# ina-foss/inaSpeechSegmenter

Measured on AMD Instinct MI355X. Metric: hours-of-audio segmented/sec (smn+gender, 16 kHz mono), higher is better.
Workload: dtype f32 (f16x3 split-operand MFMA, f32 accumulate; f64 FFT)

## Files before the change

inaspeechsegmenter_amd/_native.py:

```python
import ctypes as C
import os

import numpy as np

_HERE = os.path.dirname(os.path.abspath(__file__))
LIB_PATH = os.environ.get('ISS_LIB') or os.path.join(_HERE, 'libiss_hip.so')

PROG_COLS = 32
OP_CONV, OP_POOL, OP_SOFTMAX, OP_STATPOOL, OP_ACT, OP_ELT = 1, 2, 3, 4, 5, 6
(ELT_COPY, ELT_ADD, ELT_SUB, ELT_MUL, ELT_MAX, ELT_MIN, ELT_AVG, ELT_ZERO, ELT_PERMUTE) = range(9)
(C_OP, C_IN, C_OUT, C_RES, C_H, C_W, C_CIN, C_HO, C_WO, C_COUT, C_KH, C_KW, C_SH, C_SW, C_PT, C_PL,
 C_ACT, C_WOFF, C_BOFF, C_PSOFF, C_PTOFF, C_INMODE, C_POOLKIND, C_ORDER, C_FPOOLH, C_FPOOLW, C_DUALW, C_DUALB, C_ACTPARAM, C_ACTPARAM2, C_ACTPARAM3) = range(31)
PREC_BF16X3, PREC_F32, PREC_F16X3 = 0, 1, 2
K_ALIGN = 32
BUF_INPUT = -2
MAX_NETS = 8
RS_JOB = np.dtype([('src_offset', '<i8'), ('frames_in', '<i8'), ('channels', '<i4'), ('format', '<i4'), ('filter', '<i4'),
                   ('reserved', '<i4'), ('dst_offset', '<i8'), ('frames_out', '<i8')])
RS_FORMAT = {np.dtype(np.uint8): 0, np.dtype('<i2'): 1, np.dtype('<i4'): 2, np.dtype('<f4'): 3, np.dtype('<f8'): 4}
RS_I8, RS_ULAW, RS_ALAW, RS_SWAP = 8, 9, 10, 0x100
ADPCM_JOB = np.dtype([('src_offset', '<i8'), ('block_begin', '<i8'), ('nblocks', '<i8'), ('frames_total', '<i8'), ('channels', '<i4'),
                      ('block_align', '<i4'), ('output', '<i4'), ('filter', '<i4'), ('dst_offset', '<i8'), ('frames_out', '<i8')])
ADPCM_TO_SIGNAL, ADPCM_TO_STAGE = 0, 1
ADPCM_STATUS = {1: 'step index above 88', 2: 'predictor index above 6'}
# ... 145 lines not shown
        'iss_survey_geometry': (C.c_int, [pi32, pi32, pi32]),
        'iss_survey_stats': (C.c_int, [vp, pi64, pi64]),
        'iss_get_signal_pcm16': (C.c_int, [vp, pi16, i64, i64]),
        'iss_resample_stats': (C.c_int, [vp, pi64, pi64]),
        'iss_flac_index': (C.c_int, [vp, i64, i64, vp, vp, i64, pi64, pi64, C.c_char_p, i32]),
        'iss_flac_crc': (C.c_int, [vp, i64, pi32, pi32]),
        'iss_flac_decode_host': (C.c_int, [vp, i64, vp, i64, i32, i32, i64, vp, pi32]),
        'iss_flac_decode': (C.c_int, [vp, vp, i64, vp, i64, vp, i32, i64, pi32]),
        'iss_flac_get_stage': (C.c_int, [vp, i32, vp, i64]),
        'iss_flac_stats': (C.c_int, [vp, pi64, pi64]),
        'iss_adpcm_decode_host': (C.c_int, [vp, i64, i64, i32, i32, i64, pi16, pi32]),
        'iss_adpcm_decode': (C.c_int, [vp, vp, i64, vp, i32, i64, i64, pi32]),
        'iss_adpcm_get_stage': (C.c_int, [vp, i32, vp, i64]),
        'iss_adpcm_stats': (C.c_int, [vp, pi64, pi64]),
        'iss_msadpcm_decode_host': (C.c_int, [vp, i64, i64, i32, i32, i64, pi16, pi32]),
        'iss_msadpcm_decode': (C.c_int, [vp, vp, i64, vp, i32, i64, i64, pi32]),
        'iss_msadpcm_get_stage': (C.c_int, [vp, i32, vp, i64]),
        'iss_msadpcm_stats': (C.c_int, [vp, pi64, pi64]),
        'iss_host_alloc': (C.c_int, [vp, C.c_size_t, C.POINTER(vp)]),
        'iss_host_free': (C.c_int, [vp, vp]),
        'iss_cnn_probs_async': (C.c_int, [vp, C.c_int, pi32, i32, pf, pu8, pi64]),
        'iss_cnn_dead_stats': (C.c_int, [vp, pi64, pi64]),
        'iss_wait': (C.c_int, [vp, i64]),
        'iss_comm_unique_id': (C.c_int, [vp, pu8]),
        'iss_comm_init': (C.c_int, [vp, pu8, i32, i32]),
        'iss_comm_destroy': (C.c_int, [vp]),
        'iss_allgather_segments': (C.c_int, [vp, pi32, i32, i32, pi32, pi32]),
        'iss_comm_allreduce_max': (C.c_int, [vp, pd]),
        'iss_comm_info': (C.c_int, [vp, pi32, pi32, pi32, C.c_char_p, i32]),
        'iss_sidekit': (C.c_int, [vp, pi32]),
        'iss_get_loge': (C.c_int, [vp, pf]),
        'iss_get_mspec': (C.c_int, [vp, pf]),
        'iss_set_mspec': (C.c_int, [vp, pf, i32]),
        'iss_cnn_load': (C.c_int, [vp, C.c_int, pi32, i32, pf, i64, i32, pi64, i32, i32, i32, i32]),
        'iss_cnn_load_shared': (C.c_int, [vp, C.c_int, C.c_int, pi32, i32, i32, pi64, i32, i32, i32, i32]),
        'iss_cnn_probs': (C.c_int, [vp, C.c_int, pi32, i32, pf, pu8]),
        'iss_cnn_forward': (C.c_int, [vp, C.c_int, pf, i32, pf]),
        'iss_cnn_flops': (C.c_int, [vp, C.c_int, pd]),
        'iss_set_precision': (C.c_int, [vp, C.c_int]),
        'iss_set_precision_guard': (C.c_int, [vp, C.c_float]),
        'iss_cnn_precision_info': (C.c_int, [vp, C.c_int, pi32, pf, pi32, pi32, pf]),
        'iss_cnn_set_net_precision': (C.c_int, [vp, C.c_int, C.c_int]),
        'iss_vbx_tables': (C.c_int, [vp, pd, pd]),
        'iss_vbx_features': (C.c_int, [vp, pi32, pd, i64, pf, pi32]),
        'iss_vbx_set_dither': (C.c_int, [vp, pd, i64]),
        'iss_vbx_features_pcm16': (C.c_int, [vp, pi16, i64, pf, pi32]),
# ... 478 lines not shown
        return probs, fin.astype(bool)

    def cnn_probs_async(self, net_id, win_row, probs_out=None, finite_out=None):
        wr = np.ascontiguousarray(win_row, dtype=np.int32)
        n = wr.size
        if probs_out is None:
            probs_out = np.empty((n, self._net_out[net_id]), dtype=np.float32)
        if finite_out is None:
            finite_out = np.empty(n, dtype=np.uint8)
        assert probs_out.size >= n * self._net_out[net_id] and finite_out.size >= n
        t = C.c_int64(-1)
        self._ck(self._L.iss_cnn_probs_async(self._h, net_id, _ptr(wr, C.c_int32), n, _ptr(probs_out, C.c_float),
                                             _ptr(finite_out, C.c_uint8), C.byref(t)), 'iss_cnn_probs_async')
        return t.value, probs_out, finite_out

    def cnn_dead_stats(self):
        w, d = C.c_int64(0), C.c_int64(0)
        self._ck(self._L.iss_cnn_dead_stats(self._h, C.byref(w), C.byref(d)), 'iss_cnn_dead_stats')
        return {'windows': w.value, 'dead': d.value}

    def wait(self, ticket=-1):
        self._ck(self._L.iss_wait(self._h, int(ticket)), 'iss_wait')

    def comm_unique_id(self):
        buf = np.zeros(128, dtype=np.uint8)
        self._ck(self._L.iss_comm_unique_id(self._h, _ptr(buf, C.c_uint8)), 'iss_comm_unique_id')
        return buf.tobytes()

    def comm_init(self, uid, rank, world):
        buf = np.frombuffer(bytes(uid), dtype=np.uint8).copy()
        assert buf.size == 128
        self._ck(self._L.iss_comm_init(self._h, _ptr(buf, C.c_uint8), int(rank), int(world)), 'iss_comm_init')
        self.comm_rank, self.comm_world = int(rank), int(world)

    def comm_destroy(self):
        self._ck(self._L.iss_comm_destroy(self._h), 'iss_comm_destroy')
        self.comm_rank, self.comm_world = 0, 1

    def allgather_segments(self, rows, capacity):
        world = self.comm_world
        out = np.zeros((world, capacity, 4), dtype=np.int32)
        counts = np.zeros(world, dtype=np.int32)
        if rows is None:
            rows, n = np.zeros((1, 4), np.int32), -1
        else:
            rows = np.ascontiguousarray(rows, dtype=np.int32).reshape(-1, 4)
# ... 180 lines not shown
```

inaspeechsegmenter_amd/csrc/cnn.hip:

```cpp
#include "conv_select.h"

using namespace issk;

namespace {

template <int MODE>
__global__ __launch_bounds__(256) void conv_igemm_kernel(const ConvArgs p) {
    __shared__ __attribute__((aligned(16))) float sA[2][BM * LDK];
    __shared__ __attribute__((aligned(16))) float sB[2][BN * LDK];

    const int tid = threadIdx.x, lane = tid & 63, wv = tid >> 6;
    unsigned mt, nt;
    gemm_tile_of_block(blockIdx.x, p.nblk, p.nblk_n, mt, nt);
    const long long m0 = (long long)mt * BM;
    const int n0 = (int)nt * BN;

    const int k4 = tid & 3;
    const int lr = tid >> 2;
    RowSrc rs[2];
#pragma unroll
    for (int j = 0; j < 2; ++j) rs[j] = row_source<MODE>(p, m0 + lr + 64 * j);
    const int bn = n0 + lr;
    const bool bok = bn < p.Cout;
    const float* wrow = p.w + (size_t)(bok ? bn : 0) * p.Kpad + k4 * 4;
// ... 852 lines not shown
    if (i < n) p[i] = 0.5f;
}

__global__ void mask_probs_kernel(float* probs, const uint8_t* finite, long long n, int C) {
    const long long i = (long long)blockIdx.x * blockDim.x + threadIdx.x;
    if (i < n * C && !finite[i / C]) probs[i] = 0.5f;
}

__global__ __launch_bounds__(256) void row_flags_kernel(const float* __restrict__ mspec, int T, uint8_t* __restrict__ flag) {
    const int t = blockIdx.x * 256 + threadIdx.x;
    if (t >= T) return;
    float v[24];
#pragma unroll
    for (int k = 0; k < 6; ++k) *reinterpret_cast<float4*>(v + 4 * k) = reinterpret_cast<const float4*>(mspec + (size_t)t * 24)[k];
    flag[t] = (uint8_t)iss_row_flag(v);
}

__global__ void scatter_probs_kernel(const float* __restrict__ res, const uint8_t* __restrict__ lfinite, const int32_t* __restrict__ map,
                                     long long n, int C, float* __restrict__ out, uint8_t* __restrict__ finite) {
    const long long i = (long long)blockIdx.x * blockDim.x + threadIdx.x;
    if (i >= n * C) return;
    const long long r = i / C;
    const int k = (int)(i - r * C);
    const long long m = map[r];
    const uint8_t f = lfinite[r];
    out[m * C + k] = f ? res[i] : 0.5f;
    if (k == 0) finite[m] = f;
}

inline int roundup(int a, int b) { return (a + b - 1) / b * b; }

inline uint16_t bf16_rne(float x) {
    uint32_t u;
    memcpy(&u, &x, 4);
    u += 0x7fffu + ((u >> 16) & 1u);
    return (uint16_t)(u >> 16);
}
inline float bf16_to_f32(uint16_t h) {
    uint32_t u = (uint32_t)h << 16;
    float x;
    memcpy(&x, &u, 4);
    return x;
}

}

IssParamArrays::~IssParamArrays() {
// ... 727 lines not shown
    int chosen = eff;
    if (rc == ISS_OK) probe(eff, worst);
    const double first = worst;
    if (rc == ISS_OK && worst > (double)c->guard_threshold) {
        chosen = ISS_PREC_F32;
        const int other = eff == ISS_PREC_BF16X3 ? ISS_PREC_F16X3 : ISS_PREC_BF16X3;
        if (other == ISS_PREC_BF16X3 || n.f16_ok) {
            double w2 = 0.0;
            probe(other, w2);
            if (rc == ISS_OK && w2 <= (double)c->guard_threshold) { chosen = other; worst = w2; }
        }
    }
    c->in_guard = false;
    n.prec_override = -1;
    if (rc != ISS_OK) return rc;
    if (compared == 0) { n.guard_slots = 0; return ISS_OK; }
    n.guard_dlogp = (float)std::min(first, 1e30); n.guard_slots = compared;
    n.guard_dlogp_chosen = chosen == eff ? n.guard_dlogp : (chosen == ISS_PREC_F32 ? 0.f : (float)worst);
    if (chosen != eff) { n.prec_override = chosen; n.guard_state = ISS_GUARD_ESCALATED; }
    else n.guard_state = ISS_GUARD_PASSED;
    return ISS_OK;
}

static int ensure_row_flags(iss_ctx* c) {
    if (c->flags_epoch == c->feat_epoch) return ISS_OK;
    int rc;
    if ((rc = iss_reserve(c, c->d_rowflag, (size_t)c->T))) return rc;
    if ((rc = iss_rowflag_host(c, (size_t)c->T))) return rc;
    iss_prof_begin(c, 2, 0);
    hipLaunchKernelGGL(row_flags_kernel, dim3((c->T + 255) / 256), dim3(256), 0, c->stream, (const float*)c->mspec.p, (int)c->T,
                       (uint8_t*)c->d_rowflag.p);
    iss_prof_end(c);
    ISS_HIP(c, hipGetLastError());
    ISS_HIP(c, hipMemcpyAsync(c->h_rowflag, c->d_rowflag.p, (size_t)c->T, hipMemcpyDeviceToHost, c->stream));
    ISS_HIP(c, hipStreamSynchronize(c->stream));
    c->bad_prefix.clear();
    c->flags_epoch = c->feat_epoch;
    return ISS_OK;
}

static const std::vector<int32_t>& bad_prefix(iss_ctx* c, int w) {
    std::vector<int32_t>& P = c->bad_prefix[w];
    if (P.size() != (size_t)c->T + 1) {
        P.resize((size_t)c->T + 1);
        P[0] = 0;
        for (int32_t t = 0; t < c->T; ++t) P[t + 1] = P[t] + (c->h_rowflag[t] < w ? 1 : 0);
    }
    return P;
}

extern "C" int iss_cnn_dead_stats(iss_ctx* c, int64_t* windows, int64_t* dead) {
    if (!c) return ISS_EINVAL;
    if (windows) *windows = c->win_total;
    if (dead) *dead = c->win_dead;
    return ISS_OK;
}

static int cnn_probs_impl(iss_ctx* c, int id, const int32_t* win_row, int32_t nslots, float* probs_out,
                          uint8_t* finite_out, bool async, int64_t* ticket_out) {
    if (!c) return ISS_EINVAL;
    if (ticket_out) *ticket_out = -1;
// ... 28 lines not shown
    const bool compact = nlive < nslots;
    const int32_t* rows = compact ? lm.data() : win_row;
    if (!c->in_guard && n.guard_state == ISS_GUARD_PENDING && nlive > 0 && (rc = precision_guard(c, id, rows, nlive))) return rc;
    const size_t nup = compact ? 2 * (size_t)nlive : (size_t)nslots;
    if ((rc = iss_reserve(c, c->d_winrow, (nup ? nup : 1) * 4))) return rc;
    if ((rc = iss_reserve(c, c->d_stats, (size_t)nslots * 8))) return rc;
    if ((rc = iss_reserve(c, c->d_finite, (size_t)nslots))) return rc;
    if (compact && (rc = iss_reserve(c, c->d_lfinite, (size_t)(nlive ? nlive : 1)))) return rc;
    if ((rc = iss_reserve(c, c->d_out, (size_t)nslots * n.out_dim * 4))) return rc;
    int bc = 0;
    if (nlive > 0 && (rc = plan_chunk(c, n, nlive, &bc))) return rc;
    if (nup == 0) {
    } else if (async || compact) {
        void* pinned; int slot;
        if ((rc = iss_stage_host(c, rows, nup * 4, &pinned, &slot))) return rc;
        ISS_HIP(c, hipMemcpyAsync(c->d_winrow.p, pinned, nup * 4, hipMemcpyHostToDevice, c->stream));
        iss_stage_mark(c, slot);
    } else {
        ISS_HIP(c, hipMemcpyAsync(c->d_winrow.p, win_row, (size_t)nslots * 4, hipMemcpyHostToDevice, c->stream));
    }
    const int32_t* d_map = (const int32_t*)c->d_winrow.p + nlive;
    uint8_t* d_fin = compact ? (uint8_t*)c->d_lfinite.p : (uint8_t*)c->d_finite.p;
    const long long tot = (long long)nslots * n.out_dim;
    if (compact) {
        iss_prof_begin(c, 2, 0);
        hipLaunchKernelGGL(fill_half_kernel, dim3((unsigned)((tot + 255) / 256)), dim3(256), 0, c->stream, (float*)c->d_out.p, tot);
        iss_prof_end(c);
        ISS_HIP(c, hipGetLastError());
        ISS_HIP(c, hipMemsetAsync(c->d_finite.p, 0, (size_t)nslots, c->stream));
    }
    if (nlive > 0) {
        iss_prof_begin(c, 2, 0);
        hipLaunchKernelGGL(patch_stats_kernel, dim3((nlive + 3) / 4), dim3(256), 0, c->stream, (const float*)c->mspec.p,
                           (const int32_t*)c->d_winrow.p, nlive, n.in_w, (float*)c->d_stats.p, d_fin);
        iss_prof_end(c);
        ISS_HIP(c, hipGetLastError());
    }
    bool share = !(c->diag & ISS_DIAG_NO_SHARED_FIRST);
    if (nlive > 0) {
        int gmin = rows[0], gmax = rows[0];
        for (int i = 1; i < nlive; ++i) { gmin = std::min(gmin, rows[i]); gmax = std::max(gmax, rows[i]); }
        if ((long long)(gmax - gmin + 68) * 4 > (long long)nlive * 68) share = false;
    }
    for (int s0 = 0; s0 < nlive; s0 += bc) {
        const int cur = std::min(bc, nlive - s0);
        float* res = nullptr;
        int rmin = rows[s0], rmax = rows[s0];
        for (int i = s0 + 1; i < s0 + cur; ++i) { rmin = std::min(rmin, rows[i]); rmax = std::max(rmax, rows[i]); }
        rc = run_program(c, n, cur, (const int32_t*)c->d_winrow.p + s0, (const float*)c->d_stats.p + 2 * (size_t)s0,
                         (const uint8_t*)d_fin + s0, nullptr, &res, rmin, rmax, share);
        if (rc) return rc;
        if (compact) {
            const long long ct = (long long)cur * n.out_dim;
            iss_prof_begin(c, 2, 0);
            hipLaunchKernelGGL(scatter_probs_kernel, dim3((unsigned)((ct + 255) / 256)), dim3(256), 0, c->stream, (const float*)res,
                               (const uint8_t*)d_fin + s0, d_map + s0, (long long)cur, n.out_dim, (float*)c->d_out.p, (uint8_t*)c->d_finite.p);
            iss_prof_end(c);
            ISS_HIP(c, hipGetLastError());
        } else {
            ISS_HIP(c, hipMemcpyAsync((float*)c->d_out.p + (size_t)s0 * n.out_dim, res, (size_t)cur * n.out_dim * 4,
                                      hipMemcpyDeviceToDevice, c->stream));
        }
    }
    if (!compact) {
        hipLaunchKernelGGL(mask_probs_kernel, dim3((unsigned)((tot + 255) / 256)), dim3(256), 0, c->stream,
                           (float*)c->d_out.p, (const uint8_t*)c->d_finite.p, (long long)nslots, n.out_dim);
        ISS_HIP(c, hipGetLastError());
    }
    ISS_HIP(c, hipMemcpyAsync(probs_out, c->d_out.p, (size_t)tot * 4, hipMemcpyDeviceToHost, c->stream));
    ISS_HIP(c, hipMemcpyAsync(finite_out, c->d_finite.p, (size_t)nslots, hipMemcpyDeviceToHost, c->stream));
    if (async) {
        hipEvent_t ev;
        if (!c->ev_pool.empty()) { ev = c->ev_pool.back(); c->ev_pool.pop_back(); }
        else ISS_HIP(c, hipEventCreate(&ev));
        ISS_HIP(c, hipEventRecord(ev, c->stream));
        c->ticket_ev.push_back(ev);
        if (ticket_out) *ticket_out = c->ticket_base + (int64_t)c->ticket_ev.size() - 1;
        return ISS_OK;
    }
    ISS_HIP(c, hipStreamSynchronize(c->stream));
    iss_prof_collect(c);
    return ISS_OK;
}

extern "C" int iss_cnn_probs(iss_ctx* c, int id, const int32_t* win_row, int32_t nslots, float* probs_out,
                             uint8_t* finite_out) {
    return cnn_probs_impl(c, id, win_row, nslots, probs_out, finite_out, false, nullptr);
}

extern "C" int iss_cnn_probs_async(iss_ctx* c, int id, const int32_t* win_row, int32_t nslots, float* probs_out,
                                   uint8_t* finite_out, int64_t* ticket_out) {
    return cnn_probs_impl(c, id, win_row, nslots, probs_out, finite_out, true, ticket_out);
}

extern "C" int iss_cnn_forward(iss_ctx* c, int id, const float* x, int32_t nsamp, float* out) {
    if (!c) return ISS_EINVAL;
    if (id < 0 || id >= ISS_MAX_NETS || nsamp < 0 || (nsamp > 0 && (!x || !out)))
        return iss_fail(c, ISS_EINVAL, "iss_cnn_forward: bad argument");
    IssNet& n = c->nets[id];
    if (!n.loaded) return iss_fail(c, ISS_ESTATE, "iss_cnn_forward: net %d not loaded", id);
// ... 57 lines not shown
```

inaspeechsegmenter_amd/csrc/iss_core.cpp:

```cpp
#include "iss_internal.h"
#include <cstring>
#include <cmath>
#include <mutex>

static std::string g_err;
static std::mutex g_err_mu;

int iss_fail(iss_ctx* c, int code, const char* fmt, ...) {
    char buf[1024];
    va_list ap;
    va_start(ap, fmt);
    vsnprintf(buf, sizeof(buf), fmt, ap);
    va_end(ap);
    if (c) c->err = buf;
    else { std::lock_guard<std::mutex> l(g_err_mu); g_err = buf; }
    return code;
}

int iss_reserve(iss_ctx* c, DevBuf& b, size_t bytes) {
    if (bytes <= b.cap) return ISS_OK;
    if (b.p) { ISS_HIP(c, hipStreamSynchronize(c->stream)); ISS_HIP(c, hipFree(b.p)); b.p = nullptr; b.cap = 0; }
    size_t want = bytes + (bytes >> 3) + 256;
    hipError_t e = hipMalloc(&b.p, want);
    if (e != hipSuccess) {
// ... 38 lines not shown
    *out = c;
    return ISS_OK;
}

static void free_buf(DevBuf& b) { if (b.p) (void)hipFree(b.p); b.p = nullptr; b.cap = 0; }

extern "C" void iss_destroy(iss_ctx* c) {
    if (!c) return;
    (void)hipSetDevice(c->device);
    if (c->stream) (void)hipStreamSynchronize(c->stream);
    for (int i = 0; i < ISS_MAX_NETS; ++i) iss_cnn_free(c, i);
    void* singles[] = {c->d_window, c->d_melw, c->d_mellim, c->d_tw, c->d_vbx_window, c->d_vbx_melw, c->d_vbx_mellim};
    for (void* p : singles) if (p) (void)hipFree(p);
    DevBuf* bufs[] = {&c->sig, &c->mspec, &c->loge, &c->d_winrow, &c->d_stats, &c->d_finite, &c->d_out, &c->d_in, &c->raw1, &c->d_rowflag, &c->d_lfinite,
                      &c->vbx_sig, &c->vbx_dither, &c->vbx_fb, &c->vbx_out, &c->vbx_meta, &c->rs_src, &c->rs_jobs, &c->sv_src, &c->sv_jobs, &c->sv_ws, &c->sv_res,
                      &c->flac.src, &c->flac.rows, &c->flac.status, &c->flac.stage,
                      &c->adpcm.src, &c->adpcm.rows, &c->adpcm.status, &c->adpcm.stage,
                      &c->msadpcm.src, &c->msadpcm.rows, &c->msadpcm.status, &c->msadpcm.stage};
    for (DevBuf* b : bufs) free_buf(*b);
    for (auto& b : c->act) free_buf(b);
    for (auto& f : c->rs_filters) if (f.d_taps) (void)hipFree(f.d_taps);
    for (auto& p : c->pending) { (void)hipEventDestroy(p.a); (void)hipEventDestroy(p.b); }
    for (auto& e : c->ev_pool) (void)hipEventDestroy(e);
    for (auto& e : c->ticket_ev) (void)hipEventDestroy(e);
    for (auto& s : c->staging) { if (s.p) (void)hipHostFree(s.p); if (s.done) (void)hipEventDestroy(s.done); }
    if (c->order_ev) (void)hipEventDestroy(c->order_ev);
    if (c->h_rowflag) (void)hipHostFree(c->h_rowflag);
    iss_comm_destroy(c);
    free_buf(c->comm_send); free_buf(c->comm_recv);
    if (c->stream) (void)hipStreamDestroy(c->stream);
    delete c;
}

extern "C" int iss_set_workspace_limit(iss_ctx* c, uint64_t bytes) {
    if (!c) return ISS_EINVAL;
    if (bytes < (64ull << 20)) return iss_fail(c, ISS_EINVAL, "workspace limit below 64 MiB");
    c->ws_limit = bytes;
    return ISS_OK;
}

extern "C" int iss_synchronize(iss_ctx* c) {
    if (!c) return ISS_EINVAL;
    ISS_HIP(c, hipSetDevice(c->device));
    ISS_HIP(c, hipStreamSynchronize(c->stream));
    return ISS_OK;
}

extern "C" int iss_scribble(iss_ctx* c, uint32_t word) {
    if (!c) return ISS_EINVAL;
    ISS_HIP(c, hipSetDevice(c->device));
    ISS_HIP(c, hipStreamSynchronize(c->stream));
    std::vector<DevBuf*> bufs = {&c->raw1, &c->d_stats, &c->d_finite, &c->d_lfinite, &c->d_out, &c->d_in, &c->d_winrow, &c->d_rowflag,
                                 &c->vbx_fb, &c->vbx_meta, &c->vbx_sig, &c->rs_src, &c->rs_jobs, &c->sv_src, &c->sv_jobs, &c->sv_ws, &c->sv_res,
                                 &c->flac.src, &c->flac.rows, &c->flac.status, &c->flac.stage,
                                 &c->adpcm.src, &c->adpcm.rows, &c->adpcm.status, &c->adpcm.stage,
                                 &c->msadpcm.src, &c->msadpcm.rows, &c->msadpcm.status, &c->msadpcm.stage};
    for (auto& b : c->act) bufs.push_back(&b);
    for (DevBuf* b : bufs) {
        if (!b->p) continue;
        if (b->cap >= 4) ISS_HIP(c, hipMemsetD32Async((hipDeviceptr_t)b->p, (int)word, b->cap / 4, c->stream));
        for (size_t i = b->cap & ~(size_t)3; i < b->cap; ++i)
            ISS_HIP(c, hipMemsetD8Async((hipDeviceptr_t)((char*)b->p + i), (unsigned char)(word >> (8 * (i & 3))), 1, c->stream));
    }
    c->flags_epoch = 0;
    c->bad_prefix.clear();
    c->sv_held.id = c->flac.held = c->adpcm.held = c->msadpcm.held = 0;
    return ISS_OK;
}

extern "C" int iss_sidekit_tables(iss_ctx* c, const double* window400, const float* bank) {
    if (!c || !window400 || !bank) return iss_fail(c, ISS_EINVAL, "iss_sidekit_tables: NULL argument");
    ISS_HIP(c, hipSetDevice(c->device));
    std::vector<int32_t> lim(24 * 3);
    std::vector<float> w;
    for (int f = 0; f < 24; ++f) {
        int lo = -1, hi = -1;
        for (int k = 0; k < 257; ++k)
            if (bank[f * 257 + k] != 0.0f) { if (lo < 0) lo = k; hi = k; }
        if (lo < 0) { lo = 0; hi = -1; }
        if (hi >= 256) return iss_fail(c, ISS_EINVAL, "mel filter %d touches bin 256; unsupported table", f);
        lim[f * 3 + 0] = lo; lim[f * 3 + 1] = hi - lo + 1; lim[f * 3 + 2] = (int32_t)w.size();
        for (int k = lo; k <= hi; ++k) w.push_back(bank[f * 257 + k]);
    }
    if (w.size() > 1024) return iss_fail(c, ISS_EINVAL, "mel bank has %zu weights (>1024)", w.size());
    std::vector<double> tw(2 * 256 * 2);
    for (int k = 0; k < 256; ++k) {
        tw[2 * k] = cos(-2.0 * M_PI * k / 256.0);       tw[2 * k + 1] = sin(-2.0 * M_PI * k / 256.0);
// ... 102 lines not shown
    memcpy(c->staging[slot].p, src, bytes);
    *pinned_out = c->staging[slot].p;
    *slot_out = slot;
    return ISS_OK;
}
int iss_rowflag_host(iss_ctx* c, size_t rows) {
    if (rows <= c->h_rowflag_cap) return ISS_OK;
    if (c->h_rowflag) { ISS_HIP(c, hipStreamSynchronize(c->stream)); (void)hipHostFree(c->h_rowflag); c->h_rowflag = nullptr; c->h_rowflag_cap = 0; }
    const size_t want = rows + (rows >> 2) + 4096;
    hipError_t e = hipHostMalloc((void**)&c->h_rowflag, want, hipHostMallocDefault);
    if (e != hipSuccess) { c->h_rowflag = nullptr; return iss_fail(c, ISS_ENOMEM, "hipHostMalloc(%zu) failed: %s", want, hipGetErrorString(e)); }
    c->h_rowflag_cap = want;
    return ISS_OK;
}
void iss_stage_mark(iss_ctx* c, int slot) {
    auto& s = c->staging[slot];
    (void)hipEventRecord(s.done, c->stream);
    s.busy = true;
}

extern "C" int iss_wait(iss_ctx* c, int64_t ticket) {
    if (!c) return ISS_EINVAL;
    ISS_HIP(c, hipSetDevice(c->device));
    const int64_t last = c->ticket_base + (int64_t)c->ticket_ev.size() - 1;
    if (ticket < 0 || ticket >= last) {
        ISS_HIP(c, hipStreamSynchronize(c->stream));
        for (auto e : c->ticket_ev) c->ev_pool.push_back(e);
        c->ticket_base += (int64_t)c->ticket_ev.size();
        c->ticket_ev.clear();
        iss_prof_collect(c);
        return ISS_OK;
    }
    if (ticket < c->ticket_base) return ISS_OK;
    ISS_HIP(c, hipEventSynchronize(c->ticket_ev[(size_t)(ticket - c->ticket_base)]));
    return ISS_OK;
}

extern "C" int iss_sidekit(iss_ctx* c, int32_t* T_out) {
    if (!c) return ISS_EINVAL;
    if (!c->sk_tables) return iss_fail(c, ISS_ESTATE, "iss_sidekit: call iss_sidekit_tables first");
    if (c->sig_kind == 0) return iss_fail(c, ISS_ESTATE, "iss_sidekit: no resident signal");
    ISS_HIP(c, hipSetDevice(c->device));
    int64_t n = c->sig_n;
    int64_t T = n >= 400 ? (n - 400) / 160 + 1 : 0;
    if (T > 0x7fffffffLL / 24) return iss_fail(c, ISS_EINVAL, "signal too long (%lld frames)", (long long)T);
    c->T = (int32_t)T;
    int rc = iss_reserve(c, c->mspec, (size_t)(T > 0 ? T : 1) * 24 * sizeof(float));
    if (rc) return rc;
    rc = iss_reserve(c, c->loge, (size_t)(T > 0 ? T : 1) * sizeof(float));
    if (rc) return rc;
    if (T > 0) { rc = iss_launch_sidekit(c); if (rc) return rc; }
    c->have_feats = true; ++c->feat_epoch;
    if (T_out) *T_out = (int32_t)T;
    return ISS_OK;
}

extern "C" int iss_get_loge(iss_ctx* c, float* out) {
    if (!c || !out) return iss_fail(c, ISS_EINVAL, "iss_get_loge: NULL");
    if (!c->have_feats) return iss_fail(c, ISS_ESTATE, "iss_get_loge: no features resident");
    ISS_HIP(c, hipSetDevice(c->device));
    if (c->T > 0) ISS_HIP(c, hipMemcpyAsync(out, c->loge.p, (size_t)c->T * sizeof(float), hipMemcpyDeviceToHost, c->stream));
    ISS_HIP(c, hipStreamSynchronize(c->stream));
    iss_prof_collect(c);
    return ISS_OK;
}

extern "C" int iss_get_mspec(iss_ctx* c, float* out) {
    if (!c || !out) return iss_fail(c, ISS_EINVAL, "iss_get_mspec: NULL");
    if (!c->have_feats) return iss_fail(c, ISS_ESTATE, "iss_get_mspec: no features resident");
    ISS_HIP(c, hipSetDevice(c->device));
    if (c->T > 0) ISS_HIP(c, hipMemcpyAsync(out, c->mspec.p, (size_t)c->T * 24 * sizeof(float), hipMemcpyDeviceToHost, c->stream));
    ISS_HIP(c, hipStreamSynchronize(c->stream));
    iss_prof_collect(c);
    return ISS_OK;
}

extern "C" int iss_set_mspec(iss_ctx* c, const float* mspec, int32_t T) {
    if (!c || !mspec || T <= 0) return iss_fail(c, ISS_EINVAL, "iss_set_mspec: bad argument");
    ISS_HIP(c, hipSetDevice(c->device));
    int rc = iss_reserve(c, c->mspec, (size_t)T * 24 * sizeof(float));
    if (rc) return rc;
    ISS_HIP(c, hipMemcpyAsync(c->mspec.p, mspec, (size_t)T * 24 * sizeof(float), hipMemcpyHostToDevice, c->stream));
    ISS_HIP(c, hipStreamSynchronize(c->stream));
    c->T = T; c->have_feats = true; ++c->feat_epoch;
    if ((rc = iss_rowflag_host(c, (size_t)T))) return rc;
// ... 95 lines not shown
```

inaspeechsegmenter_amd/csrc/iss_internal.h:

```cpp
#pragma once
#include <hip/hip_runtime.h>
#include <array>
#include <cstdint>
#include <cstdio>
#include <cstdarg>
#include <string>
#include <vector>
#include <unordered_map>
#include <map>
#include <memory>
#include "../../include/iss.h"

struct DevBuf {
    void* p = nullptr;
    size_t cap = 0;
};

struct ConvOp;

struct IssCounters { int64_t launches = 0, units = 0; };
struct IssCodec {
    const char* name;
    DevBuf src, rows, status, stage;
    std::vector<int64_t> stage_off, stage_bytes;
// ... 57 lines not shown
    int sig_kind = 0;
    int64_t sig_n = 0;

    struct RsFilter { int32_t up = 1, down = 1, hl = 0; int64_t ntaps = 1; double* d_taps = nullptr; };
    std::vector<RsFilter> rs_filters;
    std::map<std::pair<int32_t, int32_t>, int32_t> rs_filter_id;
    DevBuf rs_src, rs_jobs;
    IssCounters rs_count;

    IssCodec flac{"flac"}, adpcm{"adpcm"}, msadpcm{"msadpcm"};

    DevBuf sv_src, sv_jobs, sv_ws, sv_res;
    IssCounters sv_count;
    struct Held { int64_t id = 0, bytes = 0; std::vector<iss_survey_job> jobs; std::vector<iss_set> sets; std::vector<iss_set_member> members; } sv_held;
    int64_t held_seq = 0;
    IssCounters up_count;

    DevBuf mspec, loge;
    int32_t T = 0;
    bool have_feats = false;
    uint64_t feat_epoch = 1;

    uint64_t flags_epoch = 0;
    DevBuf d_rowflag;
    uint8_t* h_rowflag = nullptr;
    size_t h_rowflag_cap = 0;
    std::map<int, std::vector<int32_t>> bad_prefix;
    DevBuf d_lfinite;
    int64_t win_total = 0, win_dead = 0;

    IssNet nets[ISS_MAX_NETS];
    uint64_t ws_limit = 24ull << 30;
    int precision = ISS_PREC_F16X3;
    float guard_threshold = 5e-4f;
    bool in_guard = false;
    uint32_t diag = 0;
    std::vector<DevBuf> act;
    DevBuf d_winrow, d_stats, d_finite, d_out, d_in;
    DevBuf raw1;

    bool vbx_tables = false;
    double* d_vbx_window = nullptr;
    double* d_vbx_melw = nullptr;
    int32_t* d_vbx_mellim = nullptr;
    DevBuf vbx_sig, vbx_dither, vbx_fb, vbx_out;
    DevBuf vbx_meta;
    int32_t vbx_T = 0;
    int64_t vbx_dither_n = 0;
    IssCounters vbx_res_count;

    struct Staging { void* p = nullptr; size_t cap = 0; hipEvent_t done = nullptr; bool busy = false; };
    std::vector<Staging> staging;
    std::vector<hipEvent_t> ticket_ev;
    int64_t ticket_base = 1;
    hipEvent_t order_ev = nullptr;

    void* comm = nullptr;
    int comm_rank = 0, comm_world = 1;
    DevBuf comm_send, comm_recv;

    bool prof = false;
    double prof_ms[ISS_PROF_KINDS] = {};
    int64_t prof_launch[ISS_PROF_KINDS] = {};
    double prof_flops[ISS_PROF_KINDS] = {};
    double prof_row_ms[ISS_PROF_ROWS] = {};
    int64_t prof_row_launch[ISS_PROF_ROWS] = {};
    struct Pending { hipEvent_t a, b; int kind; int sub; int row; double flops; std::string inst; };
    std::vector<Pending> pending;
    struct Inst { std::string name; double ms = 0; int64_t launches = 0; double flops = 0; };
    std::vector<Inst> prof_inst;
    std::vector<hipEvent_t> ev_pool;
};

int iss_fail(iss_ctx* c, int code, const char* fmt, ...);
int iss_reserve(iss_ctx* c, DevBuf& b, size_t bytes);
void iss_set_signal(iss_ctx* c, const void* ptr, int kind, int64_t n);
// ... 38 lines not shown
static_assert(sizeof(RsMixRow) == 16 && sizeof(RsTermDev) == 16 && sizeof(RsSetTermDev) == 32, "one array of 16-byte rows");
struct IssMixTables { const iss_mixset* sets; const iss_mix* mixes; int64_t nmixes; const iss_mix_term* terms; int64_t nterms; };
struct IssSetTables { const iss_set* sets; const iss_set_member* members; int64_t nmembers; };
struct IssRsPlan {
    std::vector<RsJobDev> dj;
    std::vector<RsWinDev> dw;
    std::vector<RsSplitDev> ds;
    std::vector<int32_t> sel;
    std::vector<RsMixDev> dm;
    std::vector<RsMixRow> mixes;
    std::vector<RsTermDev> terms;
    std::vector<RsSetTermDev> sterms;
    bool set = false;
    int64_t tiles = 0, lds = 0;
};
int iss_resample_plan(iss_ctx* c, const iss_resample_job* jobs, const iss_window* wins, int32_t njobs, int64_t src_bytes, int64_t nsig,
                      std::vector<std::pair<int64_t, int64_t>> ranges, const char* who, IssRsPlan& plan,
                      const iss_split* splits = nullptr, const int32_t* sel = nullptr, int64_t nsel = 0,
                      const IssMixTables* mix = nullptr, const IssSetTables* set = nullptr);
int iss_resample_launch(iss_ctx* c, const uint8_t* dev_src, const IssRsPlan& plan);

int iss_launch_sidekit(iss_ctx* c);
int iss_cnn_free(iss_ctx* c, int net_id);
```

inaspeechsegmenter_amd/segmenter.py:

```python
import os
import time
import shutil
import warnings

import threading
import weakref
import numpy as np

from . import _native
from . import tables
from . import keras_model
from . import io as iss_io
from . import resample as resample_mod
from .io import decode_pcm, _to_float
from .sources import Source, RawSource
from .export_funcs import seg2csv, seg2textgrid

_MODEL_DIRS = ('/root/.keras/inaSpeechSegmenter/', os.path.expanduser('~/.keras/inaSpeechSegmenter/'))


def pred2logemission(pred, eps=1e-10):
    pred = np.asarray(pred)
    ret = np.full((len(pred), 2), eps)
    ret[pred == 0, 0] = 1 - eps
# ... 128 lines not shown
        if st['mode'] is None:
            with st['lock']:
                if st['mode'] is None:
                    out = run()
                    info = ctx.cnn_precision_info(self.net_id)
                    if info['state'] in ('passed', 'escalated'):
                        st['mode'] = self._MODES[info['mode']]
                        st['told'].add(id(ctx))
                    elif info['state'] == 'fixed' or not _guard_on(ctx):
                        st['mode'] = -1
                    return out
        if st['mode'] >= 0 and id(ctx) not in st['told']:
            with st['lock']:
                if id(ctx) not in st['told']:
                    if ctx.cnn_precision_info(self.net_id)['state'] == 'pending':
                        ctx.cnn_set_net_precision(self.net_id, st['mode'])
                        st['pinned'][id(ctx)] = ctx
                    st['told'].add(id(ctx))
        return run()

    def __call__(self, mspec, lseg, difflen=0, dense=False, ctx=None, allpred=None):
        ctx = ctx or self.ctx
        nframes = _ensure_resident(ctx, mspec)
        rows = _window_rows(nframes, difflen)
        todo = [(start, stop) for lab, start, stop in lseg if lab == self.inlabel]
        if todo:
            idx = np.concatenate([np.arange(s, e) for s, e in todo])
            if allpred is not None:
                rawpred = allpred[idx]
            elif dense:
                allpred, _finite = self.probs(ctx, rows)
                rawpred = allpred[idx]
            else:
                rawpred, _finite = self.probs(ctx, rows[idx])
        ret = []
        trans = diag_trans_exp(self.viterbi_arg, len(self.outlabels))
        pos = 0
        for lab, start, stop in lseg:
            if lab != self.inlabel:
                ret.append((lab, start, stop))
                continue
            n = stop - start
            r = rawpred[pos:pos + n]
            pos += n
            with np.errstate(divide='ignore'):
                pred = viterbi_decoding(np.log(r), trans)
            for lab2, start2, stop2 in _binidx2seglist(pred):
                ret.append((self.outlabels[int(lab2)], start2 + start, stop2 + start))
        return ret


class SpeechMusic(DnnSegmenter):
    outlabels = ('speech', 'music')
    model_fname = 'keras_speech_music_cnn.hdf5'
    inlabel = 'energy'
    nmel = 21
    viterbi_arg = 150
    net_id = 0


class SpeechMusicNoise(DnnSegmenter):
    outlabels = ('speech', 'music', 'noise')
    model_fname = 'keras_speech_music_noise_cnn.hdf5'
    inlabel = 'energy'
    nmel = 21
    viterbi_arg = 80
    net_id = 0


class Gender(DnnSegmenter):
    outlabels = ('female', 'male')
# ... 119 lines not shown
        elif vad_engine == 'smn':
            self.vad = SpeechMusicNoise(batch_size, self.ctx, models)

        assert detect_gender in [True, False]
        self.detect_gender = detect_gender
        if detect_gender:
            self.gender = Gender(batch_size, self.ctx, models)

    def close(self):
        from . import pipeline
        pipeline.close_workers(self)

    def segment_slots(self, mspec, loge, difflen, dense=False):
        pending = None
        if dense and self.detect_gender:
            ctx = self.ctx
            rows = _window_rows(_ensure_resident(ctx, mspec), difflen)
            t1, p1, _ = self.vad.probs(ctx, rows, async_out=self._pinned_out(0, len(rows), len(self.vad.outlabels)))
            t2, p2, _ = self.gender.probs(ctx, rows, async_out=self._pinned_out(1, len(rows), len(self.gender.outlabels)))
            pending = (t1, p1, t2, p2)
        lseg = _energy_segments(loge, self.energy_ratio)
        if pending is not None:
            t1, p1, t2, p2 = pending
            self.ctx.wait(t1)
            lseg = self.vad(mspec, lseg, difflen, allpred=p1)
            self.ctx.wait(t2)
            return self.gender(mspec, lseg, difflen, allpred=p2)
        lseg = self.vad(mspec, lseg, difflen, dense=dense)
        if self.detect_gender:
            lseg = self.gender(mspec, lseg, difflen, dense=dense)
        return lseg

    def _pinned_out(self, k, n, c):
        cache = self.__dict__.setdefault('_pin_out', {})
        cur = cache.get(k)
        if cur is None or cur[0].shape[0] < n or cur[0].shape[1] != c:
            if cur is not None:
                self.ctx.pinned_free(cur[0]); self.ctx.pinned_free(cur[1])
            cap = int(n * 1.1) + 64
            cur = (self.ctx.pinned_empty((cap, c), np.float32), self.ctx.pinned_empty((cap,), np.uint8))
            cache[k] = cur
        return cur[0][:n], cur[1][:n]

    def segment_feats(self, mspec, loge, difflen, start_sec):
        lseg = self.segment_slots(mspec, loge, difflen)
        return [(lab, start_sec + start * .02, start_sec + stop * .02) for lab, start, stop in lseg]

    def segment_device_pcm(self, dev_ptr, n, dense=False):
        if n < 400 + 160 * 67:
            raise ValueError("segment_device_pcm needs at least 68 frames (use segment_signal for short media)")
# ... 374 lines not shown
```

include/iss.h:

```cpp
#ifndef ISS_H
#define ISS_H

#include <stdint.h>
#include <stddef.h>

#ifdef __cplusplus
extern "C" {
#endif

#define ISS_OK        0
#define ISS_EINVAL   -1
#define ISS_ENODEV   -2
#define ISS_EHIP     -3
#define ISS_ESTATE   -4
#define ISS_ENOMEM   -5
#define ISS_ETIMEOUT -6

typedef struct iss_ctx iss_ctx;

int         iss_create(int device_id, iss_ctx** out);
void        iss_destroy(iss_ctx* ctx);
const char* iss_last_error(const iss_ctx* ctx);
const char* iss_version(void);
int         iss_set_workspace_limit(iss_ctx* ctx, uint64_t bytes);
// ... 270 lines not shown
    ISS_C_ORDER,
    ISS_C_FPOOLH, ISS_C_FPOOLW,
    ISS_C_DUALW, ISS_C_DUALB,
    ISS_C_ACTPARAM,
    ISS_C_ACTPARAM2, ISS_C_ACTPARAM3,
};
#define ISS_BUF_INPUT  (-2)

int iss_cnn_load(iss_ctx* ctx, int net_id, const int32_t* prog, int32_t nrows,
                 const float* blob, int64_t blob_floats,
                 int32_t nbuf, const int64_t* buf_elems,
                 int32_t in_h, int32_t in_w, int32_t in_c, int32_t out_dim);
int iss_cnn_load_shared(iss_ctx* ctx, int net_id, int src_id, const int32_t* prog, int32_t nrows,
                        int32_t nbuf, const int64_t* buf_elems,
                        int32_t in_h, int32_t in_w, int32_t in_c, int32_t out_dim);

int iss_cnn_probs(iss_ctx* ctx, int net_id, const int32_t* win_row, int32_t n,
                  float* probs_out , uint8_t* finite_out );

int iss_cnn_probs_async(iss_ctx* ctx, int net_id, const int32_t* win_row, int32_t n,
                        float* probs_out , uint8_t* finite_out , int64_t* ticket_out);
int iss_cnn_dead_stats(iss_ctx* ctx, int64_t* windows, int64_t* dead);
int iss_wait(iss_ctx* ctx, int64_t ticket);

int iss_cnn_forward(iss_ctx* ctx, int net_id, const float* x, int32_t n, float* out );

#define ISS_PREC_BF16X3 0
#define ISS_PREC_F32    1
#define ISS_PREC_F16X3  2
int iss_set_precision(iss_ctx* ctx, int mode);

#define ISS_GUARD_PENDING   0
#define ISS_GUARD_PASSED    1
#define ISS_GUARD_ESCALATED 2
#define ISS_GUARD_FIXED     3
int iss_set_precision_guard(iss_ctx* ctx, float threshold);
int iss_cnn_precision_info(iss_ctx* ctx, int id, int32_t* mode, float* max_dlogp, int32_t* slots, int32_t* state, float* dlogp_in_use);
int iss_cnn_set_net_precision(iss_ctx* ctx, int id, int mode);

#define ISS_DIAG_NO_SHARED_FIRST 0x001u
#define ISS_DIAG_NO_FLROWS       0x002u
#define ISS_DIAG_NO_WS           0x004u
#define ISS_DIAG_NO_WS3          0x008u
#define ISS_DIAG_NO_DIRECT1      0x010u
#define ISS_DIAG_NO_NH2          0x020u
#define ISS_DIAG_NO_TR           0x040u
// ... 76 lines not shown
```

Baseline: 7.396.

## Stream CNN probs per batch pass into pinned memory and smooth landed spans incrementally

Async CNN probability output is now written straight into pinned host memory by the scatter kernel after each batch pass, with an event recorded per pass. A new iss_wait_slots call lets the host wait only until the slots it needs have arrived, and host-side Viterbi smoothing runs span by span while later passes are still computing. Row-flag computation is also queued right after feature extraction so it overlaps other work instead of requiring a separate sync later. The cost is more events, zero-copy device writes over PCIe or fabric, host-side filling of dead slots, and more complex ticket bookkeeping.

```diff
diff --git a/inaspeechsegmenter_amd/_native.py b/inaspeechsegmenter_amd/_native.py
--- a/inaspeechsegmenter_amd/_native.py
+++ b/inaspeechsegmenter_amd/_native.py
@@ -191,6 +191,7 @@
         'iss_cnn_probs_async': (C.c_int, [vp, C.c_int, pi32, i32, pf, pu8, pi64]),
         'iss_cnn_dead_stats': (C.c_int, [vp, pi64, pi64]),
         'iss_wait': (C.c_int, [vp, i64]),
+        'iss_wait_slots': (C.c_int, [vp, i64, i32, pi32]),
         'iss_comm_unique_id': (C.c_int, [vp, pu8]),
         'iss_comm_init': (C.c_int, [vp, pu8, i32, i32]),
         'iss_comm_destroy': (C.c_int, [vp]),
@@ -715,6 +716,11 @@
     def wait(self, ticket=-1):
         self._ck(self._L.iss_wait(self._h, int(ticket)), 'iss_wait')
 
+    def wait_slots(self, ticket, upto):
+        landed = C.c_int32(0)
+        self._ck(self._L.iss_wait_slots(self._h, int(ticket), int(upto), C.byref(landed)), 'iss_wait_slots')
+        return landed.value
+
     def comm_unique_id(self):
         buf = np.zeros(128, dtype=np.uint8)
         self._ck(self._L.iss_comm_unique_id(self._h, _ptr(buf, C.c_uint8)), 'iss_comm_unique_id')
diff --git a/inaspeechsegmenter_amd/csrc/cnn.hip b/inaspeechsegmenter_amd/csrc/cnn.hip
--- a/inaspeechsegmenter_amd/csrc/cnn.hip
+++ b/inaspeechsegmenter_amd/csrc/cnn.hip
@@ -898,7 +898,7 @@
     if (i >= n * C) return;
     const long long r = i / C;
     const int k = (int)(i - r * C);
-    const long long m = map[r];
+    const long long m = map ? map[r] : r;
     const uint8_t f = lfinite[r];
     out[m * C + k] = f ? res[i] : 0.5f;
     if (k == 0) finite[m] = f;
@@ -1672,8 +1672,8 @@
     return ISS_OK;
 }
 
-static int ensure_row_flags(iss_ctx* c) {
-    if (c->flags_epoch == c->feat_epoch) return ISS_OK;
+int iss_enqueue_row_flags(iss_ctx* c) {
+    if (c->T <= 0) return ISS_OK;
     int rc;
     if ((rc = iss_reserve(c, c->d_rowflag, (size_t)c->T))) return rc;
     if ((rc = iss_rowflag_host(c, (size_t)c->T))) return rc;
@@ -1683,10 +1683,26 @@
     iss_prof_end(c);
     ISS_HIP(c, hipGetLastError());
     ISS_HIP(c, hipMemcpyAsync(c->h_rowflag, c->d_rowflag.p, (size_t)c->T, hipMemcpyDeviceToHost, c->stream));
+    return ISS_OK;
+}
+
+static int ensure_row_flags(iss_ctx* c) {
+    if (c->flags_epoch == c->feat_epoch) return ISS_OK;
+    int rc;
+    if (c->flags_queued != c->feat_epoch && (rc = iss_enqueue_row_flags(c))) return rc;
     ISS_HIP(c, hipStreamSynchronize(c->stream));
     c->bad_prefix.clear();
     c->flags_epoch = c->feat_epoch;
     return ISS_OK;
+}
+
+static bool host_pinned(const void* p, size_t bytes) {
+    for (const char* q : {(const char*)p, (const char*)p + (bytes ? bytes - 1 : 0)}) {
+        hipPointerAttribute_t at;
+        if (hipPointerGetAttributes(&at, q) != hipSuccess) { (void)hipGetLastError(); return false; }
+        if (at.type != hipMemoryTypeHost) return false;
+    }
+    return true;
 }
 
 static const std::vector<int32_t>& bad_prefix(iss_ctx* c, int w) {
@@ -1761,7 +1777,19 @@
     const int32_t* d_map = (const int32_t*)c->d_winrow.p + nlive;
     uint8_t* d_fin = compact ? (uint8_t*)c->d_lfinite.p : (uint8_t*)c->d_finite.p;
     const long long tot = (long long)nslots * n.out_dim;
-    if (compact) {
+    float* dev_probs = nullptr;
+    uint8_t* dev_finite = nullptr;
+    const bool per_pass = async && !c->in_guard &&
+                          host_pinned(probs_out, (size_t)tot * 4) && host_pinned(finite_out, (size_t)nslots) &&
+                          hipHostGetDevicePointer((void**)&dev_probs, probs_out, 0) == hipSuccess &&
+                          hipHostGetDevicePointer((void**)&dev_finite, finite_out, 0) == hipSuccess;
+    if (per_pass && compact) {
+        for (int i = 0, j = 0; i < nslots; ++i) {
+            if (j < nlive && lm[(size_t)nlive + j] == i) { ++j; continue; }
+            for (int k = 0; k < n.out_dim; ++k) probs_out[(size_t)i * n.out_dim + k] = 0.5f;
+            finite_out[i] = 0;
+        }
+    } else if (compact) {
         iss_prof_begin(c, 2, 0);
         hipLaunchKernelGGL(fill_half_kernel, dim3((unsigned)((tot + 255) / 256)), dim3(256), 0, c->stream, (float*)c->d_out.p, tot);
         iss_prof_end(c);
@@ -1781,6 +1809,17 @@
         for (int i = 1; i < nlive; ++i) { gmin = std::min(gmin, rows[i]); gmax = std::max(gmax, rows[i]); }
         if ((long long)(gmax - gmin + 68) * 4 > (long long)nlive * 68) share = false;
     }
+    iss_ctx::Ticket ticket;
+    auto landing = [&](int32_t end) -> int {
+        if (!async) return ISS_OK;
+        hipEvent_t ev;
+        if (!c->ev_pool.empty()) { ev = c->ev_pool.back(); c->ev_pool.pop_back(); }
+        else ISS_HIP(c, hipEventCreate(&ev));
+        ticket.land.push_back({end, ev});
+        ISS_HIP(c, hipEventRecord(ev, c->stream));
+        return ISS_OK;
+    };
+    auto give_back = [&]() { for (auto& l : ticket.land) c->ev_pool.push_back(l.ev); ticket.land.clear(); };
     for (int s0 = 0; s0 < nlive; s0 += bc) {
         const int cur = std::min(bc, nlive - s0);
         float* res = nullptr;
@@ -1788,33 +1827,36 @@
         for (int i = s0 + 1; i < s0 + cur; ++i) { rmin = std::min(rmin, rows[i]); rmax = std::max(rmax, rows[i]); }
         rc = run_program(c, n, cur, (const int32_t*)c->d_winrow.p + s0, (const float*)c->d_stats.p + 2 * (size_t)s0,
                          (const uint8_t*)d_fin + s0, nullptr, &res, rmin, rmax, share);
-        if (rc) return rc;
-        if (compact) {
+        if (rc) { give_back(); return rc; }
+        if (compact || per_pass) {
             const long long ct = (long long)cur * n.out_dim;
+            float* out = per_pass ? dev_probs : (float*)c->d_out.p;
+            uint8_t* fin = per_pass ? dev_finite : (uint8_t*)c->d_finite.p;
             iss_prof_begin(c, 2, 0);
             hipLaunchKernelGGL(scatter_probs_kernel, dim3((unsigned)((ct + 255) / 256)), dim3(256), 0, c->stream, (const float*)res,
-                               (const uint8_t*)d_fin + s0, d_map + s0, (long long)cur, n.out_dim, (float*)c->d_out.p, (uint8_t*)c->d_finite.p);
+                               (const uint8_t*)d_fin + s0, compact ? d_map + s0 : (const int32_t*)nullptr, (long long)cur, n.out_dim,
+                               compact ? out : out + (size_t)s0 * n.out_dim, compact ? fin : fin + s0);
             iss_prof_end(c);
-            ISS_HIP(c, hipGetLastError());
+            if (hipGetLastError() != hipSuccess) { give_back(); return iss_fail(c, ISS_EHIP, "scatter_probs_kernel launch failed"); }
         } else {
             ISS_HIP(c, hipMemcpyAsync((float*)c->d_out.p + (size_t)s0 * n.out_dim, res, (size_t)cur * n.out_dim * 4,
                                       hipMemcpyDeviceToDevice, c->stream));
         }
-    }
-    if (!compact) {
-        hipLaunchKernelGGL(mask_probs_kernel, dim3((unsigned)((tot + 255) / 256)), dim3(256), 0, c->stream,
-                           (float*)c->d_out.p, (const uint8_t*)c->d_finite.p, (long long)nslots, n.out_dim);
-        ISS_HIP(c, hipGetLastError());
-    }
-    ISS_HIP(c, hipMemcpyAsync(probs_out, c->d_out.p, (size_t)tot * 4, hipMemcpyDeviceToHost, c->stream));
-    ISS_HIP(c, hipMemcpyAsync(finite_out, c->d_finite.p, (size_t)nslots, hipMemcpyDeviceToHost, c->stream));
+        if (per_pass && (rc = landing(s0 + cur >= nlive ? nslots : (compact ? lm[(size_t)nlive + s0 + cur] : s0 + cur)))) { give_back(); return rc; }
+    }
+    if (!per_pass) {
+        if (!compact) {
+            hipLaunchKernelGGL(mask_probs_kernel, dim3((unsigned)((tot + 255) / 256)), dim3(256), 0, c->stream,
+                               (float*)c->d_out.p, (const uint8_t*)c->d_finite.p, (long long)nslots, n.out_dim);
+            ISS_HIP(c, hipGetLastError());
+        }
+        ISS_HIP(c, hipMemcpyAsync(probs_out, c->d_out.p, (size_t)tot * 4, hipMemcpyDeviceToHost, c->stream));
+        ISS_HIP(c, hipMemcpyAsync(finite_out, c->d_finite.p, (size_t)nslots, hipMemcpyDeviceToHost, c->stream));
+    }
+    if ((!per_pass || nlive == 0) && (rc = landing(nslots))) { give_back(); return rc; }
     if (async) {
-        hipEvent_t ev;
-        if (!c->ev_pool.empty()) { ev = c->ev_pool.back(); c->ev_pool.pop_back(); }
-        else ISS_HIP(c, hipEventCreate(&ev));
-        ISS_HIP(c, hipEventRecord(ev, c->stream));
-        c->ticket_ev.push_back(ev);
-        if (ticket_out) *ticket_out = c->ticket_base + (int64_t)c->ticket_ev.size() - 1;
+        c->tickets.push_back(std::move(ticket));
+        if (ticket_out) *ticket_out = c->ticket_base + (int64_t)c->tickets.size() - 1;
         return ISS_OK;
     }
     ISS_HIP(c, hipStreamSynchronize(c->stream));
diff --git a/inaspeechsegmenter_amd/csrc/iss_core.cpp b/inaspeechsegmenter_amd/csrc/iss_core.cpp
--- a/inaspeechsegmenter_amd/csrc/iss_core.cpp
+++ b/inaspeechsegmenter_amd/csrc/iss_core.cpp
@@ -84,7 +84,7 @@
     for (auto& f : c->rs_filters) if (f.d_taps) (void)hipFree(f.d_taps);
     for (auto& p : c->pending) { (void)hipEventDestroy(p.a); (void)hipEventDestroy(p.b); }
     for (auto& e : c->ev_pool) (void)hipEventDestroy(e);
-    for (auto& e : c->ticket_ev) (void)hipEventDestroy(e);
+    for (auto& t : c->tickets) for (auto& l : t.land) (void)hipEventDestroy(l.ev);
     for (auto& s : c->staging) { if (s.p) (void)hipHostFree(s.p); if (s.done) (void)hipEventDestroy(s.done); }
     if (c->order_ev) (void)hipEventDestroy(c->order_ev);
     if (c->h_rowflag) (void)hipHostFree(c->h_rowflag);
@@ -124,7 +124,7 @@
         for (size_t i = b->cap & ~(size_t)3; i < b->cap; ++i)
             ISS_HIP(c, hipMemsetD8Async((hipDeviceptr_t)((char*)b->p + i), (unsigned char)(word >> (8 * (i & 3))), 1, c->stream));
     }
-    c->flags_epoch = 0;
+    c->flags_epoch = c->flags_queued = 0;
     c->bad_prefix.clear();
     c->sv_held.id = c->flac.held = c->adpcm.held = c->msadpcm.held = 0;
     return ISS_OK;
@@ -273,17 +273,39 @@
 extern "C" int iss_wait(iss_ctx* c, int64_t ticket) {
     if (!c) return ISS_EINVAL;
     ISS_HIP(c, hipSetDevice(c->device));
-    const int64_t last = c->ticket_base + (int64_t)c->ticket_ev.size() - 1;
+    const int64_t last = c->ticket_base + (int64_t)c->tickets.size() - 1;
     if (ticket < 0 || ticket >= last) {
         ISS_HIP(c, hipStreamSynchronize(c->stream));
-        for (auto e : c->ticket_ev) c->ev_pool.push_back(e);
-        c->ticket_base += (int64_t)c->ticket_ev.size();
-        c->ticket_ev.clear();
+        for (auto& t : c->tickets) for (auto& l : t.land) c->ev_pool.push_back(l.ev);
+        c->ticket_base += (int64_t)c->tickets.size();
+        c->tickets.clear();
         iss_prof_collect(c);
         return ISS_OK;
     }
     if (ticket < c->ticket_base) return ISS_OK;
-    ISS_HIP(c, hipEventSynchronize(c->ticket_ev[(size_t)(ticket - c->ticket_base)]));
+    ISS_HIP(c, hipEventSynchronize(c->tickets[(size_t)(ticket - c->ticket_base)].land.back().ev));
+    return ISS_OK;
+}
+
+extern "C" int iss_wait_slots(iss_ctx* c, int64_t ticket, int32_t upto, int32_t* landed_out) {
+    if (!c || !landed_out) return iss_fail(c, ISS_EINVAL, "iss_wait_slots: NULL argument");
+    *landed_out = 0x7fffffff;
+    if (ticket < c->ticket_base || ticket >= c->ticket_base + (int64_t)c->tickets.size()) return ISS_OK;
+    ISS_HIP(c, hipSetDevice(c->device));
+    auto& t = c->tickets[(size_t)(ticket - c->ticket_base)];
+    const auto& land = t.land;
+    if (upto > 0 && (t.done == 0 || (land[t.done - 1].slot_end < upto && t.done < land.size()))) {
+        size_t k = t.done;
+        while (k + 1 < land.size() && land[k].slot_end < upto) ++k;
+        ISS_HIP(c, hipEventSynchronize(land[k].ev));
+        t.done = k + 1;
+    }
+    for (; t.done < land.size(); ++t.done) {
+        const hipError_t e = hipEventQuery(land[t.done].ev);
+        if (e == hipErrorNotReady) break;
+        if (e != hipSuccess) return iss_fail(c, ISS_EHIP, "hipEventQuery failed: %s", hipGetErrorString(e));
+    }
+    *landed_out = t.done ? land[t.done - 1].slot_end : 0;
     return ISS_OK;
 }
 
@@ -302,6 +324,10 @@
     if (rc) return rc;
     if (T > 0) { rc = iss_launch_sidekit(c); if (rc) return rc; }
     c->have_feats = true; ++c->feat_epoch;
+    if (T > 0) {
+        if ((rc = iss_enqueue_row_flags(c))) return rc;
+        c->flags_queued = c->feat_epoch;
+    }
     if (T_out) *T_out = (int32_t)T;
     return ISS_OK;
 }
@@ -312,6 +338,10 @@
     ISS_HIP(c, hipSetDevice(c->device));
     if (c->T > 0) ISS_HIP(c, hipMemcpyAsync(out, c->loge.p, (size_t)c->T * sizeof(float), hipMemcpyDeviceToHost, c->stream));
     ISS_HIP(c, hipStreamSynchronize(c->stream));
+    if (c->flags_queued == c->feat_epoch && c->flags_epoch != c->feat_epoch) {
+        c->bad_prefix.clear();
+        c->flags_epoch = c->feat_epoch;
+    }
     iss_prof_collect(c);
     return ISS_OK;
 }
diff --git a/inaspeechsegmenter_amd/csrc/iss_internal.h b/inaspeechsegmenter_amd/csrc/iss_internal.h
--- a/inaspeechsegmenter_amd/csrc/iss_internal.h
+++ b/inaspeechsegmenter_amd/csrc/iss_internal.h
@@ -103,6 +103,7 @@
     uint64_t feat_epoch = 1;
 
     uint64_t flags_epoch = 0;
+    uint64_t flags_queued = 0;
     DevBuf d_rowflag;
     uint8_t* h_rowflag = nullptr;
     size_t h_rowflag_cap = 0;
@@ -132,7 +133,9 @@
 
     struct Staging { void* p = nullptr; size_t cap = 0; hipEvent_t done = nullptr; bool busy = false; };
     std::vector<Staging> staging;
-    std::vector<hipEvent_t> ticket_ev;
+    struct Landing { int32_t slot_end; hipEvent_t ev; };
+    struct Ticket { std::vector<Landing> land; size_t done = 0; };
+    std::vector<Ticket> tickets;
     int64_t ticket_base = 1;
     hipEvent_t order_ev = nullptr;
 
@@ -217,3 +220,4 @@
 
 int iss_launch_sidekit(iss_ctx* c);
 int iss_cnn_free(iss_ctx* c, int net_id);
+int iss_enqueue_row_flags(iss_ctx* c);
diff --git a/inaspeechsegmenter_amd/segmenter.py b/inaspeechsegmenter_amd/segmenter.py
--- a/inaspeechsegmenter_amd/segmenter.py
+++ b/inaspeechsegmenter_amd/segmenter.py
@@ -174,17 +174,16 @@
     def __call__(self, mspec, lseg, difflen=0, dense=False, ctx=None, allpred=None):
         ctx = ctx or self.ctx
         nframes = _ensure_resident(ctx, mspec)
-        rows = _window_rows(nframes, difflen)
         todo = [(start, stop) for lab, start, stop in lseg if lab == self.inlabel]
         if todo:
             idx = np.concatenate([np.arange(s, e) for s, e in todo])
             if allpred is not None:
                 rawpred = allpred[idx]
             elif dense:
-                allpred, _finite = self.probs(ctx, rows)
+                allpred, _finite = self.probs(ctx, _window_rows(nframes, difflen))
                 rawpred = allpred[idx]
             else:
-                rawpred, _finite = self.probs(ctx, rows[idx])
+                rawpred, _finite = self.probs(ctx, _window_rows(nframes, difflen)[idx])
         ret = []
         trans = diag_trans_exp(self.viterbi_arg, len(self.outlabels))
         pos = 0
@@ -199,6 +198,46 @@
                 pred = viterbi_decoding(np.log(r), trans)
             for lab2, start2, stop2 in _binidx2seglist(pred):
                 ret.append((self.outlabels[int(lab2)], start2 + start, stop2 + start))
+        return ret
+
+    def smooth_landed(self, ctx, ticket, allpred, lseg):
+        spans = [(start, stop) for lab, start, stop in lseg if lab == self.inlabel]
+        if not spans:
+            return list(lseg)
+        trans = diag_trans_exp(self.viterbi_arg, len(self.outlabels))
+        wait_slots = getattr(ctx, 'wait_slots', None)
+        runs = [[] for _ in spans]
+        i = 0
+        while i < len(spans):
+            if wait_slots is None:
+                ctx.wait(ticket)
+                landed = len(allpred)
+            else:
+                landed = wait_slots(ticket, spans[i][1])
+            j = i + 1
+            while j < len(spans) and spans[j][1] <= landed:
+                j += 1
+            first = np.array([s for s, _ in spans[i:j]], dtype=np.int64)
+            length = np.array([e - s for s, e in spans[i:j]], dtype=np.int64)
+            with np.errstate(divide='ignore'):
+                em = np.log(allpred[spans[i][0]:spans[i][1]] if j == i + 1 else
+                            np.concatenate([allpred[s:e] for s, e in spans[i:j]]))
+            pred = _native.viterbi_segments(em, length, trans)
+            off = np.concatenate(([0], np.cumsum(length)))
+            a = np.union1d(np.flatnonzero(pred[1:] != pred[:-1]) + 1, off[:-1])
+            b = np.append(a[1:], len(pred))
+            k = np.searchsorted(off, a, side='right') - 1
+            shift = first[k] - off[k]
+            for lab, kk, s, e in zip(pred[a].tolist(), k.tolist(), (a + shift).tolist(), (b + shift).tolist()):
+                runs[i + kk].append((self.outlabels[lab], s, e))
+            i = j
+        ret, k = [], 0
+        for seg in lseg:
+            if seg[0] != self.inlabel:
+                ret.append(seg)
+            else:
+                ret.extend(runs[k])
+                k += 1
         return ret
 
 
@@ -364,10 +403,10 @@
         lseg = _energy_segments(loge, self.energy_ratio)
         if pending is not None:
             t1, p1, t2, p2 = pending
-            self.ctx.wait(t1)
-            lseg = self.vad(mspec, lseg, difflen, allpred=p1)
+            lseg = self.vad.smooth_landed(self.ctx, t1, p1, lseg)
+            lseg = self.gender.smooth_landed(self.ctx, t2, p2, lseg)
             self.ctx.wait(t2)
-            return self.gender(mspec, lseg, difflen, allpred=p2)
+            return lseg
         lseg = self.vad(mspec, lseg, difflen, dense=dense)
         if self.detect_gender:
             lseg = self.gender(mspec, lseg, difflen, dense=dense)
diff --git a/include/iss.h b/include/iss.h
--- a/include/iss.h
+++ b/include/iss.h
@@ -316,6 +316,7 @@
                         float* probs_out , uint8_t* finite_out , int64_t* ticket_out);
 int iss_cnn_dead_stats(iss_ctx* ctx, int64_t* windows, int64_t* dead);
 int iss_wait(iss_ctx* ctx, int64_t ticket);
+int iss_wait_slots(iss_ctx* ctx, int64_t ticket, int32_t upto, int32_t* landed_out);
 
 int iss_cnn_forward(iss_ctx* ctx, int net_id, const float* x, int32_t n, float* out );
 
```

Result: faster. 7.545 (median of 6 runs) (+2.0%).
